# microsoft/ORBIT-Dataset

Hardware: AMD Instinct MI355X
Metric: query frames/sec per task (224×224, 5-way ProtoNet) + frame accuracy vs ref (higher is better)
Workload: dtype f32

## Files before the change

### orbit-dataset_amd/csrc/mbconv_rows.hip

```cpp
#include "bf3.h"
#include "common.h"

namespace orbit {

using f32x16 = __attribute__((ext_vector_type(16))) float;
using v4f = __attribute__((ext_vector_type(4))) float;

using v2f = __attribute__((ext_vector_type(2))) float;

__device__ __forceinline__ v2f silu2(v2f x) {
    const v2f t = x * (v2f){-1.44269502f, -1.44269502f};
    const v2f e = {__builtin_amdgcn_exp2f(t.x), __builtin_amdgcn_exp2f(t.y)};
    const v2f d = e + (v2f){1.0f, 1.0f};
    const v2f r = {__builtin_amdgcn_rcpf(d.x), __builtin_amdgcn_rcpf(d.y)};
    return x * r;
}
__device__ __forceinline__ v2f fma2(v2f a, v2f b, v2f c) { return __builtin_elementwise_fma(a, b, c); }

struct MbRowsParams {
    const float* x;
    const float* w1;
    const float* sc1;
    const float* sh1;
    const float* wdw;
    const float* sc2;
    const float* sh2;
    float* y;
    float* pool;
    int H, W, Cin, mid, pad_t, pad_l, Ho, Wo;
    int SWo, SWi, strips, band_rows, bands, nchunk, total;
};

constexpr int ROWS_ES = 36;

template <int K, int S, int TO, int NOUT, int NG, int SPR, bool EXACT, bool BF3, bool RAW = false>
__global__ __launch_bounds__(256, K == 3 ? 3 : 2) void mbconv_rows3_kernel(const MbRowsParams p) {
    constexpr int NEW = TO * S;
    constexpr int NCOL = (NOUT - 1) * S + K;
    constexpr int ES = ROWS_ES;
    static_assert((TO - 1) * S + K <= 2 * NEW, "an output step reads two windows");
    static_assert(NEW <= 4, "row-in-window index is packed in 2 bits");

    extern __shared__ __attribute__((aligned(16))) float smem[];
    const int n_new = NEW * p.SWi;
    float* ring = smem;

    const int per = gridDim.x >> 3;
    const int v = (blockIdx.x & 7) * per + (blockIdx.x >> 3);
    if (v >= p.total) return;
    const int chunk = v % p.nchunk;
    const int t = v / p.nchunk;
    const int tiles = p.strips * p.bands;
    const int tile = t % tiles, b = t / tiles;
    const int strip = tile % p.strips, band = tile / p.strips;

    const int tid = threadIdx.x, lane = tid & 63;
    const int wave = __builtin_amdgcn_readfirstlane(tid >> 6);
    const int l31 = lane & 31, lh = lane >> 5;
    const int c0 = chunk * 32;
    const int x0 = strip * p.SWo, y0 = band * p.band_rows;
    const int y1 = y0 + p.band_rows < p.Ho ? y0 + p.band_rows : p.Ho;
    const int wi0 = x0 * S - p.pad_l;
    const int r_first = y0 * S - p.pad_t;
    const int NI = (y1 - y0 + TO - 1) / TO;

    const int tstart = wave * 32 < n_new - 32 ? wave * 32 : n_new - 32;
    int a_off, a_rl;
    bool a_colok;
    {
        const int f = tstart + l31;
        a_rl = f / p.SWi;
        const int col = f - a_rl * p.SWi, wi = wi0 + col;
        a_colok = (unsigned)wi < (unsigned)p.W;
        a_off = (a_rl * p.W + wi) * p.Cin + 4 * lh;
    }
    unsigned rowsel[NEW];
#pragma unroll
    for (int r = 0; r < NEW; ++r) rowsel[r] = 0;
#pragma unroll
    for (int e = 0; e < 16; ++e) {
        const int f = tstart + 8 * (e >> 2) + 4 * lh + (e & 3);
        const int rl = f / p.SWi, col = f - rl * p.SWi;
        const bool cok = (unsigned)(wi0 + col) < (unsigned)p.W;
#pragma unroll
        for (int r = 0; r < NEW; ++r)
            if (cok && rl == r) rowsel[r] |= 1u << e;
    }
    v4f wb[NG];
    float s1 = 0.f, h1 = 0.f;
    {
        const int ch = c0 + l31;
#pragma unroll
        for (int g = 0; g < NG; ++g) {
            wb[g] = (v4f){0.f, 0.f, 0.f, 0.f};
            if (ch < p.mid) wb[g] = *reinterpret_cast<const v4f*>(p.w1 + (size_t)ch * p.Cin + 8 * g + 4 * lh);
        }
        if (ch < p.mid) s1 = p.sc1[ch], h1 = p.sh1[ch];
    }
    uint2 wq[BF3 ? 3 : 1][BF3 ? NG : 1];
    if constexpr (BF3) {
#pragma unroll
        for (int g = 0; g < NG; ++g) split3(wb[g], wq[0][g], wq[1][g], wq[2][g]);
    }
    const float* xb = p.x + (size_t)b * p.H * p.W * p.Cin;
    v4f xa[NG];
    auto load_x = [&](int w) {
        const int hi0 = r_first + w * NEW;
        const bool ok = a_colok && (unsigned)(hi0 + a_rl) < (unsigned)p.H;
        const float* src = ok ? xb + (ptrdiff_t)hi0 * p.W * p.Cin + a_off : xb + 4 * lh;
#pragma unroll
        for (int g = 0; g < NG; ++g) xa[g] = *reinterpret_cast<const v4f*>(src + 8 * g);
    };
    float* const Ew0 = ring + tstart * ES + l31;
    auto expand = [&](int w, int slot3) {
        float* Ew = Ew0 + slot3 * n_new * ES;
        const int hi0 = r_first + w * NEW;
        unsigned rowmask = 0;
#pragma unroll
        for (int r = 0; r < NEW; ++r) rowmask |= ((unsigned)(hi0 + r) < (unsigned)p.H ? 1u : 0u) << r;
        f32x16 acc;
#pragma unroll
        for (int r = 0; r < 16; ++r) acc[r] = 0.f;
        if (rowmask != 0) {
            if constexpr (BF3) {
                const uint2 z2 = {0u, 0u};
#pragma unroll
                for (int g = 0; g < NG; g += 2) {
                    uint2 xq[3][2];
                    split3(xa[g], xq[0][0], xq[1][0], xq[2][0]);
                    if (g + 1 < NG) split3(xa[g + 1], xq[0][1], xq[1][1], xq[2][1]);
                    else xq[0][1] = xq[1][1] = xq[2][1] = z2;
                    bf16x8 af[3], bf[3];
#pragma unroll
                    for (int q = 0; q < 3; ++q) {
                        af[q] = bf3_frag(xq[q][0], xq[q][1]);
                        bf[q] = bf3_frag(wq[q][g], g + 1 < NG ? wq[q][g + 1] : z2);
                    }
                    acc = __builtin_amdgcn_mfma_f32_32x32x16_bf16(af[2], bf[0], acc, 0, 0, 0);
                    acc = __builtin_amdgcn_mfma_f32_32x32x16_bf16(af[0], bf[2], acc, 0, 0, 0);
                    acc = __builtin_amdgcn_mfma_f32_32x32x16_bf16(af[1], bf[1], acc, 0, 0, 0);
                    acc = __builtin_amdgcn_mfma_f32_32x32x16_bf16(af[1], bf[0], acc, 0, 0, 0);
                    acc = __builtin_amdgcn_mfma_f32_32x32x16_bf16(af[0], bf[1], acc, 0, 0, 0);
                    acc = __builtin_amdgcn_mfma_f32_32x32x16_bf16(af[0], bf[0], acc, 0, 0, 0);
                }
            } else {
#pragma unroll
                for (int g = 0; g < NG; ++g)
#pragma unroll
                    for (int kk = 0; kk < 4; ++kk) acc = __builtin_amdgcn_mfma_f32_32x32x2f32(xa[g][kk], wb[g][kk], acc, 0, 0, 0);
            }
        }
        load_x(w + 1 <= NI ? w + 1 : NI);
        unsigned okbits = 0;
#pragma unroll
        for (int r = 0; r < NEW; ++r) okbits |= ((rowmask >> r) & 1u) ? rowsel[r] : 0u;
        const v2f s1v = {s1, s1}, h1v = {h1, h1};
        if (__all(okbits == 0xffffu)) {
#pragma unroll
            for (int e = 0; e < 16; e += 2) {
                const v2f val = silu2(fma2((v2f){acc[e], acc[e + 1]}, s1v, h1v));
                Ew[(8 * (e >> 2) + 4 * lh + (e & 3)) * ES] = val.x;
                Ew[(8 * (e >> 2) + 4 * lh + (e & 3) + 1) * ES] = val.y;
            }
        } else {
#pragma unroll
            for (int e = 0; e < 16; e += 2) {
                const v2f val = silu2(fma2((v2f){acc[e], acc[e + 1]}, s1v, h1v));
                const int m0 = __builtin_amdgcn_sbfe((int)okbits, e, 1), m1 = __builtin_amdgcn_sbfe((int)okbits, e + 1, 1);
                const float vx = val.x, vy = val.y;
                Ew[(8 * (e >> 2) + 4 * lh + (e & 3)) * ES] = __int_as_float(__float_as_int(vx) & m0);
                Ew[(8 * (e >> 2) + 4 * lh + (e & 3) + 1) * ES] = __int_as_float(__float_as_int(vy) & m1);
            }
        }
    };

    static_assert(NOUT * S == 2 || NOUT * S == 4, "lane map is built for a 2- or 4-pixel item pitch");
    const unsigned long long CHUNK_MAP = NOUT * S == 2 ? 0xFDCE5764B98A1320ull : 0xFDCE9BA875461320ull;
    const int ck = (int)((CHUNK_MAP >> (4 * (lane >> 2))) & 15u);
    const int lc = ((ck & 1) << 2) | (lane & 3);
    const int u = wave * 8 + (ck >> 1);
    const bool q_real = c0 + lc * 4 < p.mid;
    const int lce = EXACT && !q_real ? lc - 4 : lc;
    const int cq = c0 + lce * 4;
    const bool q_ok = EXACT || q_real;
    static_assert(TO % (32 / SPR) == 0, "a pass covers whole rows of the step");
    v4f s2 = {0.f, 0.f, 0.f, 0.f}, h2 = {0.f, 0.f, 0.f, 0.f};
    if (!RAW && q_ok) s2 = *reinterpret_cast<const v4f*>(p.sc2 + cq), h2 = *reinterpret_cast<const v4f*>(p.sh2 + cq);
    v4f* Ds = reinterpret_cast<v4f*>(ring + 3 * n_new * ES);
    v4f tapr[K == 3 ? K * K : 1];
    if constexpr (K == 3) {
#pragma unroll
        for (int tap = 0; tap < K * K; ++tap)
            tapr[tap] = q_ok ? *reinterpret_cast<const v4f*>(p.wdw + (size_t)tap * p.mid + cq) : (v4f){0.f, 0.f, 0.f, 0.f};
    } else if (tid < K * K * 8) {
        const int tq = c0 + (tid & 7) * 4;
        Ds[tid] = tq < p.mid ? *reinterpret_cast<const v4f*>(p.wdw + (size_t)(tid >> 3) * p.mid + tq) : (v4f){0.f, 0.f, 0.f, 0.f};
    }
    constexpr int RPP = 32 / SPR;
    constexpr int NPASS = (TO + RPP - 1) / RPP;
    const int G = p.SWo / NOUT;
    const int jl = u / SPR, g = u % SPR;
    const int gc = g < G ? g : G - 1;
    const int rowfl = p.SWi * ES;
    const int colpart = gc * (NOUT * S * ES) + lce * 4;
    const int o_col = (x0 + gc * NOUT) * p.mid + cq;
    unsigned okn = 0;
#pragma unroll
    for (int n = 0; n < NOUT; ++n)
        if (g < G && q_ok && x0 + g * NOUT + n < p.Wo) okn |= 1u << n;
    const bool own = g < G && q_real;
    float* ystep = p.y + ((size_t)b * p.Ho + y0) * p.Wo * p.mid;
    const int ystride = TO * p.Wo * p.mid;
    const int orow = p.Wo * p.mid;
    const int band_len = y1 - y0;
    const int winfl = n_new * ES;
    v4f psum = {0.f, 0.f, 0.f, 0.f}, psq = {0.f, 0.f, 0.f, 0.f};

    auto depthwise = [&](int i, int slotA) {
        const int baseA = slotA * winfl;
        const int baseB = slotA == 2 ? 0 : baseA + winfl;
        v2f alo[NOUT], ahi[NOUT];
        v4f cA[NCOL], cB[NCOL];
        auto fetch = [&](v4f* c, int pass, int kh) {
            const float* erow;
            if constexpr (RPP == 1) {
                const int rr = pass * S + kh;
                erow = ring + ((rr >= NEW ? baseB + (rr - NEW) * rowfl : baseA + rr * rowfl) + colpart);
            } else {
                const int rr = (pass * RPP + jl) * S + kh;
                erow = ring + ((rr >= NEW ? baseB - NEW * rowfl : baseA) + __mul24(rr, rowfl) + colpart);
            }
#pragma unroll
            for (int q = 0; q < NCOL; ++q) c[q] = *reinterpret_cast<const v4f*>(erow + q * ES);
        };
        auto mac = [&](const v4f* c, const v4f* t) {
#pragma unroll
            for (int kw = 0; kw < K; ++kw) {
                const v2f flo = {t[kw][0], t[kw][1]}, fhi = {t[kw][2], t[kw][3]};
#pragma unroll
                for (int n = 0; n < NOUT; ++n) {
                    const v4f cv = c[n * S + kw];
                    alo[n] = fma2((v2f){cv[0], cv[1]}, flo, alo[n]);
                    ahi[n] = fma2((v2f){cv[2], cv[3]}, fhi, ahi[n]);
                }
            }
        };
        fetch(cA, 0, 0);
#pragma unroll
        for (int pass = 0; pass < NPASS; ++pass) {
#pragma unroll
            for (int n = 0; n < NOUT; ++n) alo[n] = (v2f){0.f, 0.f}, ahi[n] = (v2f){0.f, 0.f};
            if constexpr (K == 3) {
#pragma unroll
                for (int kh = 0; kh < K; ++kh) {
                    const int f = pass * K + kh;
                    v4f* cur = (f & 1) ? cB : cA;
                    v4f* nxt = (f & 1) ? cA : cB;
                    if (kh + 1 < K) fetch(nxt, pass, kh + 1);
                    else if (pass + 1 < NPASS) fetch(nxt, pass + 1, 0);
                    mac(cur, tapr + kh * K);
                }
            } else {
                static_assert(K == 3 || NPASS == 1, "the 5x5 row loop assumes one pass");
                v4f tA[K], tB[K];
                auto taps = [&](v4f* t, int kh) {
#pragma unroll
                    for (int kw = 0; kw < K; ++kw) t[kw] = Ds[(kh * K + kw) * 8 + lce];
                };
                taps(tA, 0);
#pragma unroll 1
                for (int kh = 0; kh + 1 < K; kh += 2) {
                    fetch(cB, pass, kh + 1), taps(tB, kh + 1);
                    mac(cA, tA);
                    if (kh + 2 < K) fetch(cA, pass, kh + 2), taps(tA, kh + 2);
                    mac(cB, tB);
                }
                if (K & 1) mac(cA, tA);
            }
            const int j = pass * RPP + jl;
            const bool rowok = j < TO && i * TO + j < band_len;
            float* yrow = ystep + j * orow;
#pragma unroll
            for (int n = 0; n < NOUT; ++n) {
                if constexpr (RAW) {
                    const v4f o = {alo[n].x, alo[n].y, ahi[n].x, ahi[n].y};
                    const bool mine = EXACT ? own : (rowok && ((okn >> n) & 1u));
                    if (EXACT || mine) *reinterpret_cast<v4f*>(yrow + (o_col + n * p.mid)) = o;
                    {
#pragma clang fp contract(off)
                        const v4f z = {0.f, 0.f, 0.f, 0.f};
                        psum = psum + (mine ? o : z);
                        psq = psq + (mine ? o * o : z);
                    }
                } else if constexpr (EXACT) {
                    const v2f olo = silu2(fma2(alo[n], (v2f){s2[0], s2[1]}, (v2f){h2[0], h2[1]}));
                    const v2f ohi = silu2(fma2(ahi[n], (v2f){s2[2], s2[3]}, (v2f){h2[2], h2[3]}));
                    const v4f o = {olo.x, olo.y, ohi.x, ohi.y};
                    *reinterpret_cast<v4f*>(yrow + (o_col + n * p.mid)) = o;
                    psum += own ? o : (v4f){0.f, 0.f, 0.f, 0.f};
                } else if (rowok && ((okn >> n) & 1u)) {
                    const v2f olo = silu2(fma2(alo[n], (v2f){s2[0], s2[1]}, (v2f){h2[0], h2[1]}));
                    const v2f ohi = silu2(fma2(ahi[n], (v2f){s2[2], s2[3]}, (v2f){h2[2], h2[3]}));
                    const v4f o = {olo.x, olo.y, ohi.x, ohi.y};
                    *reinterpret_cast<v4f*>(yrow + (o_col + n * p.mid)) = o;
                    {
#pragma clang fp contract(off)
                        psum = psum + o;
                    }
                }
            }
        }
        ystep += ystride;
    };

    load_x(0);
    expand(0, 0);
    expand(1, 1);
    __syncthreads();
    __builtin_amdgcn_s_waitcnt(0x0F70);
    int sa = 0;
    for (int i = 0; i < NI; ++i) {
        if (i + 2 <= NI) expand(i + 2, sa == 0 ? 2 : sa - 1);
        depthwise(i, sa);
        sa = sa == 2 ? 0 : sa + 1;
        __syncthreads();
    }
    if (p.pool) {
        v4f* red = reinterpret_cast<v4f*>(ring);
        red[u * 8 + lc] = psum;
        if constexpr (RAW) red[256 + u * 8 + lc] = psq;
        __syncthreads();
        if (tid < 8 && c0 + tid * 4 < p.mid) {
            v4f t4 = red[tid];
            for (int sl = 1; sl < 32; ++sl) t4 += red[sl * 8 + tid];
            if constexpr (RAW) {
                v4f q4 = red[256 + tid];
                for (int sl = 1; sl < 32; ++sl) q4 += red[256 + sl * 8 + tid];
                float* row = p.pool + ((size_t)b * tiles + tile) * 2 * p.mid + c0 + tid * 4;
                *reinterpret_cast<v4f*>(row) = t4;
                *reinterpret_cast<v4f*>(row + p.mid) = q4;
            } else {
                *reinterpret_cast<v4f*>(p.pool + ((size_t)b * tiles + tile) * p.mid + c0 + tid * 4) = t4;
            }
        }
    }
}

struct RowsGeom {
    int SWo, SWi, strips, band_rows, bands, TO, NOUT;
};
static bool rows_geom(int H, int W, int Cin, int mid, int K, int stride, int Ho, int Wo, RowsGeom& g) {
    if (Cin % 8 != 0 || mid % 4 != 0 || H < 1 || W < 1) return false;
    const int ng = Cin / 8;
    int swo_max = 0;
    if (K == 3 && stride == 2 && ng == 2) g.TO = 1, g.NOUT = 1, swo_max = 28;
    else if (K == 3 && stride == 1 && ng == 3) g.TO = 2, g.NOUT = 2, swo_max = 56;
    else if (K == 5 && stride == 2 && ng == 3) g.TO = 2, g.NOUT = 1, swo_max = 14;
    else if (K == 5 && stride == 1 && ng == 5) g.TO = 4, g.NOUT = 4, swo_max = 28;
    else if (K == 3 && stride == 2 && ng == 5) g.TO = 2, g.NOUT = 1, swo_max = 14;
    else return false;
    g.strips = cdiv(Wo, swo_max);
    g.SWo = cdiv(cdiv(Wo, g.strips), g.NOUT) * g.NOUT;
    g.SWi = (g.SWo - 1) * stride + K;
    const int n_new = g.TO * stride * g.SWi;
    if (n_new <= 32 || n_new > 128) return false;
    g.band_rows = 28;
    g.band_rows = cdiv(g.band_rows, g.TO) * g.TO;
    g.bands = cdiv(Ho, g.band_rows);
    return true;
}

bool mbconv_rows_supported(int H, int W, int Cin, int mid, int K, int stride) {
    RowsGeom g;
    const int Ho = cdiv(H, stride), Wo = cdiv(W, stride);
    return rows_geom(H, W, Cin, mid, K, stride, Ho, Wo, g);
}

int mbconv_rows_tiles(int H, int W, int Cin, int mid, int K, int stride) {
    RowsGeom g;
    const int Ho = cdiv(H, stride), Wo = cdiv(W, stride);
    if (!rows_geom(H, W, Cin, mid, K, stride, Ho, Wo, g)) return 0;
    return g.strips * g.bands;
}

int launch_mbconv_rows(const float* x, const float* w1, const float* sc1, const float* sh1, const float* wdw,
                       const float* sc2, const float* sh2, float* y, float* pool, int B, int H, int W, int Cin, int mid,
                       int K, int stride, int pad_t, int pad_l, int Ho, int Wo, hipStream_t s, int plan_tiles, bool raw_stats) {
    ORBIT_REQUIRE(x && w1 && sc1 && sh1 && wdw && y && (raw_stats ? pool != nullptr : (sc2 && sh2)), "mbconv_rows: null pointer");
    RowsGeom g;
    ORBIT_REQUIRE(Ho == cdiv(H, stride) && Wo == cdiv(W, stride) && rows_geom(H, W, Cin, mid, K, stride, Ho, Wo, g),
                  "mbconv_rows: unsupported shape (H=%d W=%d Cin=%d mid=%d K=%d s=%d)", H, W, Cin, mid, K, stride);
    ORBIT_REQUIRE(plan_tiles <= 0 || plan_tiles == g.strips * g.bands,
                  "mbconv_rows: the plan was built for %d pooling tiles per frame, this launch writes %d", plan_tiles, g.strips * g.bands);
    MbRowsParams p;
    p.x = x, p.w1 = w1, p.sc1 = sc1, p.sh1 = sh1, p.wdw = wdw, p.sc2 = sc2, p.sh2 = sh2, p.y = y, p.pool = pool;
    p.H = H, p.W = W, p.Cin = Cin, p.mid = mid, p.pad_t = pad_t, p.pad_l = pad_l, p.Ho = Ho, p.Wo = Wo;
    p.SWo = g.SWo, p.SWi = g.SWi, p.strips = g.strips, p.band_rows = g.band_rows, p.bands = g.bands;
    p.nchunk = cdiv(mid, 32);
    p.total = p.nchunk * g.strips * g.bands * B;
    const int grid = cdiv(p.total, 8) * 8;
    const int n_new = g.TO * stride * g.SWi;
    const size_t lds = (size_t)3 * n_new * ROWS_ES * sizeof(float) + (K == 3 ? 0 : (size_t)K * K * 8 * 16);
    const double pix = (double)B * H * W;
    const int rec = prof_start(raw_stats ? "mbconv_rows,raw" : "mbconv_rows", 2.0 * pix * Cin * mid + 2.0 * B * Ho * Wo * mid * K * K,
                               4.0 * (pix * Cin + (double)B * Ho * Wo * mid), s, pix * mid + (raw_stats ? 0.0 : (double)B * Ho * Wo * mid));
#define ORBIT_MBR3(KK, SS, TO_, NOUT_, NG_, SPR_, EX_, BF_)                                                       \
    do {                                                                                                \
        if (raw_stats) {                                                                                \
            if constexpr (!BF_) {                                                                       \
                auto kern = mbconv_rows3_kernel<KK, SS, TO_, NOUT_, NG_, SPR_, EX_, false, true>;           \
                static bool attr_set = false;                                                           \
                if (!attr_set) {                                                                        \
                    ORBIT_HIP_CHECK(hipFuncSetAttribute(reinterpret_cast<const void*>(kern),            \
                                                        hipFuncAttributeMaxDynamicSharedMemorySize, 64 * 1024)); \
                    attr_set = true;                                                                    \
                }                                                                                       \
                kern<<<grid, 256, lds, s>>>(p);                                                         \
            }                                                                                           \
            break;                                                                                      \
        }                                                                                               \
        auto kern = mbconv_rows3_kernel<KK, SS, TO_, NOUT_, NG_, SPR_, EX_, BF_>;                                \
        static bool attr_set = false;                                                                   \
        if (!attr_set) {                                                                                \
            ORBIT_HIP_CHECK(hipFuncSetAttribute(reinterpret_cast<const void*>(kern),                    \
                                                hipFuncAttributeMaxDynamicSharedMemorySize, 64 * 1024)); \
            attr_set = true;                                                                            \
        }                                                                                               \
        kern<<<grid, 256, lds, s>>>(p);                                                                 \
    } while (0)
    const int ng = Cin / 8;
    const bool exact = g.strips * g.SWo == Wo && Ho % g.TO == 0 && g.band_rows % g.TO == 0 && (mid % 32 == 0 || mid % 32 == 16) &&
                       g.SWo % g.NOUT == 0;
    const bool bf3 = !raw_stats && (get_option("conv_bf3") & 2) != 0;
#define ORBIT_MBR3X(KK, SS, TO_, NOUT_, NG_, SPR_)                    \
    do {                                                              \
        if (exact && bf3) ORBIT_MBR3(KK, SS, TO_, NOUT_, NG_, SPR_, true, true);   \
        else if (exact) ORBIT_MBR3(KK, SS, TO_, NOUT_, NG_, SPR_, true, false);    \
        else ORBIT_MBR3(KK, SS, TO_, NOUT_, NG_, SPR_, false, false);              \
    } while (0)
    if (K == 3 && stride == 2 && ng == 2) ORBIT_MBR3X(3, 2, 1, 1, 2, 32);
    else if (K == 3 && stride == 1 && ng == 3) ORBIT_MBR3X(3, 1, 2, 2, 3, 32);
    else if (K == 5 && stride == 2 && ng == 3) ORBIT_MBR3X(5, 2, 2, 1, 3, 16);
    else if (K == 5 && stride == 1 && ng == 5) ORBIT_MBR3X(5, 1, 4, 4, 5, 8);
    else if (exact) ORBIT_MBR3(3, 2, 2, 1, 5, 16, true, false);
    else ORBIT_MBR3(3, 2, 2, 1, 5, 16, false, false);
#undef ORBIT_MBR3X
#undef ORBIT_MBR3
    prof_stop(rec, s);
    ORBIT_LAUNCH_CHECK();
    return ORBIT_OK;
}


struct StemRowsParams {
    const float* frames;
    const float* w1;
    const float* sc1;
    const float* sh1;
    const float* wdw;
    const float* sc2;
    const float* sh2;
    float* y;
    float* pool;
    int FH, FW, spad_t, spad_l, H, W;
    int SWo, SWi, strips, band_rows, bands, total;
};

constexpr int STEM_PW = 64;

template <bool EXACT>
__global__ __launch_bounds__(256, 3) void stem_rows_kernel(const StemRowsParams p, const float* __restrict__ w1g,
                                                           const float* __restrict__ sc1g, const float* __restrict__ sh1g) {
    constexpr int K = 3, TO = 2, NEW = 2, NOUT = 2, NCOL = 4, ES = ROWS_ES;
    extern __shared__ __attribute__((aligned(16))) float smem[];
    const int n_new = NEW * p.SWi;
    float* ring = smem;
    float* patch = ring + 3 * n_new * ES;
    constexpr int PATCH = 3 * 5 * STEM_PW;

    const int per = gridDim.x >> 3;
    const int v = (blockIdx.x & 7) * per + (blockIdx.x >> 3);
    if (v >= p.total) return;
    const int tiles = p.strips * p.bands;
    const int tile = v % tiles, b = v / tiles;
    const int strip = tile % p.strips, band = tile / p.strips;
    const int tid = threadIdx.x, lane = tid & 63;
    const int wave = __builtin_amdgcn_readfirstlane(tid >> 6);
    const int x0 = strip * p.SWo, y0 = band * p.band_rows;
    const int y1 = y0 + p.band_rows < p.H ? y0 + p.band_rows : p.H;
    const int c_first = x0 - 1, r_first = y0 - 1;
    const int NI = (y1 - y0 + TO - 1) / TO;
    const float* fb = p.frames + (size_t)b * 3 * p.FH * p.FW;

    const int fcol0 = 2 * c_first - p.spad_l;
    const int pcols = 2 * p.SWi + 1;
    constexpr int NPL = (PATCH + 255) / 256;
    float preg[NPL];
    unsigned pmask = 0;
    int poff[NPL];
    unsigned pcolok = 0, prows = 0;
#pragma unroll
    for (int u = 0; u < NPL; ++u) {
        const int i = tid + u * 256;
        const int c = i & (STEM_PW - 1), pr = i >> 6;
        const int plane = pr / 5, row = pr - plane * 5;
        const int fc = fcol0 + c;
        const bool cok = i < PATCH && c < pcols && (unsigned)fc < (unsigned)p.FW;
        poff[u] = cok ? (plane * p.FH + row) * p.FW + fc : 0;
        pcolok |= (cok ? 1u : 0u) << u;
        prows |= (unsigned)row << (3 * u);
    }
    auto patch_load = [&](int w) {
        const int frow0 = 2 * (r_first + NEW * w) - p.spad_t;
        unsigned rmask = 0;
#pragma unroll
        for (int r = 0; r < 5; ++r) rmask |= ((unsigned)(frow0 + r) < (unsigned)p.FH ? 1u : 0u) << r;
        const int rowbase = frow0 * p.FW;
        pmask = 0;
#pragma unroll
        for (int u = 0; u < NPL; ++u) {
            const bool ok = ((pcolok >> u) & 1u) && ((rmask >> ((prows >> (3 * u)) & 7u)) & 1u);
            pmask |= (ok ? 1u : 0u) << u;
            preg[u] = fb[ok ? poff[u] + rowbase : 0];
        }
    };
    auto patch_store = [&](int w) {
        float* dst = patch + (w & 1) * PATCH;
#pragma unroll
        for (int u = 0; u < NPL; ++u) {
            const int i = tid + u * 256;
            if (i < PATCH) dst[i] = ((pmask >> u) & 1u) ? preg[u] : 0.f;
        }
    };

    using f32x4 = __attribute__((ext_vector_type(4))) float;
    const int l15 = lane & 15, lq = lane >> 4;
    float* Wl = patch + 2 * PATCH;
    for (int i = tid; i < 14 * 64; i += 256) {
        const int ln = i & 63, hs = i >> 6, h = hs / 7, st = hs - h * 7;
        const int k = 4 * st + (ln >> 4);
        Wl[i] = k < 27 ? w1g[(16 * h + (ln & 15)) * 32 + k] : 0.f;
    }
    int a_base;
    {
        const int fa = wave * 16 + l15 < n_new ? wave * 16 + l15 : n_new - 1;
        const int rl = fa / p.SWi, col = fa - rl * p.SWi;
        a_base = (2 * rl) * STEM_PW + 2 * col;
    }
    float s1c[2], h1c[2];
#pragma unroll
    for (int h = 0; h < 2; ++h) s1c[h] = sc1g[16 * h + l15], h1c[h] = sh1g[16 * h + l15];
    unsigned o_inwin = 0, sel0 = 0, sel1 = 0;
#pragma unroll
    for (int r = 0; r < 4; ++r) {
        const int fo = wave * 16 + 4 * lq + r;
        const int rl = fo / p.SWi, col = fo - rl * p.SWi;
        if (fo < n_new) o_inwin |= 1u << r;
        if (fo < n_new && (unsigned)(c_first + col) < (unsigned)p.W) (rl ? sel1 : sel0) |= 1u << r;
    }
    auto stem = [&](int w) {
        const float* P = patch + (w & 1) * PATCH + a_base;
        f32x4 acc0 = {0.f, 0.f, 0.f, 0.f}, acc1 = {0.f, 0.f, 0.f, 0.f};
#pragma unroll
        for (int st = 0; st < 7; ++st) {
            const int k = 4 * st + lq < 27 ? 4 * st + lq : 0;
            const int ci = k / 9, kh = (k - ci * 9) / 3, kw = k - ci * 9 - kh * 3;
            const float av = P[(ci * 5 + kh) * STEM_PW + kw];
            acc0 = __builtin_amdgcn_mfma_f32_16x16x4f32(av, Wl[st * 64 + lane], acc0, 0, 0, 0);
            acc1 = __builtin_amdgcn_mfma_f32_16x16x4f32(av, Wl[(7 + st) * 64 + lane], acc1, 0, 0, 0);
        }
        const int hi0 = r_first + NEW * w;
        const unsigned okbits = ((unsigned)hi0 < (unsigned)p.H ? sel0 : 0u) | ((unsigned)(hi0 + 1) < (unsigned)p.H ? sel1 : 0u);
        float* E = ring + ((w % 3) * n_new + wave * 16 + 4 * lq) * ES + l15;
#pragma unroll
        for (int r = 0; r < 4; r += 2) {
            const v2f v0 = silu2(fma2((v2f){acc0[r], acc0[r + 1]}, (v2f){s1c[0], s1c[0]}, (v2f){h1c[0], h1c[0]}));
            const v2f v1 = silu2(fma2((v2f){acc1[r], acc1[r + 1]}, (v2f){s1c[1], s1c[1]}, (v2f){h1c[1], h1c[1]}));
            const float a0 = v0.x, a1 = v0.y, b0 = v1.x, b1 = v1.y;
            const int m0 = __builtin_amdgcn_sbfe((int)okbits, r, 1), m1 = __builtin_amdgcn_sbfe((int)okbits, r + 1, 1);
            if ((o_inwin >> r) & 1u) {
                E[r * ES] = __int_as_float(__float_as_int(a0) & m0);
                E[r * ES + 16] = __int_as_float(__float_as_int(b0) & m0);
            }
            if ((o_inwin >> (r + 1)) & 1u) {
                E[(r + 1) * ES] = __int_as_float(__float_as_int(a1) & m1);
                E[(r + 1) * ES + 16] = __int_as_float(__float_as_int(b1) & m1);
            }
        }
    };

    const unsigned long long CHUNK_MAP = 0xFDCE5764B98A1320ull;
    const int ck = (int)((CHUNK_MAP >> (4 * (lane >> 2))) & 15u);
    const int lc = ((ck & 1) << 2) | (lane & 3);
    const int u = wave * 8 + (ck >> 1);
    const int cq = lc * 4;
    const v4f s2 = *reinterpret_cast<const v4f*>(p.sc2 + cq), h2 = *reinterpret_cast<const v4f*>(p.sh2 + cq);
    v4f tapr[K * K];
#pragma unroll
    for (int tap = 0; tap < K * K; ++tap) tapr[tap] = *reinterpret_cast<const v4f*>(p.wdw + tap * 32 + cq);
    const int G = p.SWo / NOUT;
    const int jl = u >> 4, g = u & 15;
    const int gc = g < G ? g : G - 1;
    const int rowfl = p.SWi * ES, winfl = n_new * ES;
    const int colpart = gc * (NOUT * ES) + lc * 4;
    const int o_col = (jl * p.W + x0 + gc * NOUT) * 32 + cq;
    const bool own = g < G;
    unsigned okn = 0;
#pragma unroll
    for (int n = 0; n < NOUT; ++n)
        if (g < G && x0 + g * NOUT + n < p.W) okn |= 1u << n;
    float* ystep = p.y + ((size_t)b * p.H + y0) * p.W * 32;
    const int band_len = y1 - y0;
    v4f psum = {0.f, 0.f, 0.f, 0.f};
    auto depthwise = [&](int i, int slotA) {
        const int baseA = slotA * winfl;
        const int baseB = slotA == 2 ? 0 : baseA + winfl;
        v2f alo[NOUT], ahi[NOUT];
#pragma unroll
        for (int n = 0; n < NOUT; ++n) alo[n] = (v2f){0.f, 0.f}, ahi[n] = (v2f){0.f, 0.f};
        v4f cA[NCOL], cB[NCOL];
        auto fetch = [&](v4f* c, int kh) {
            const int rr = jl + kh;
            const float* erow = ring + ((rr >= NEW ? baseB - NEW * rowfl : baseA) + __mul24(rr, rowfl) + colpart);
#pragma unroll
            for (int q = 0; q < NCOL; ++q) c[q] = *reinterpret_cast<const v4f*>(erow + q * ES);
        };
        fetch(cA, 0);
#pragma unroll
        for (int kh = 0; kh < K; ++kh) {
            v4f* cur = (kh & 1) ? cB : cA;
            v4f* nxt = (kh & 1) ? cA : cB;
            if (kh + 1 < K) fetch(nxt, kh + 1);
#pragma unroll
            for (int kw = 0; kw < K; ++kw) {
                const v4f t = tapr[kh * K + kw];
                const v2f flo = {t[0], t[1]}, fhi = {t[2], t[3]};
#pragma unroll
                for (int n = 0; n < NOUT; ++n) {
                    const v4f cv = cur[n + kw];
                    alo[n] = fma2((v2f){cv[0], cv[1]}, flo, alo[n]);
                    ahi[n] = fma2((v2f){cv[2], cv[3]}, fhi, ahi[n]);
                }
            }
        }
        const bool rowok = i * TO + jl < band_len;
#pragma unroll
        for (int n = 0; n < NOUT; ++n) {
            if constexpr (EXACT) {
                const v2f olo = silu2(fma2(alo[n], (v2f){s2[0], s2[1]}, (v2f){h2[0], h2[1]}));
                const v2f ohi = silu2(fma2(ahi[n], (v2f){s2[2], s2[3]}, (v2f){h2[2], h2[3]}));
                const v4f o = {olo.x, olo.y, ohi.x, ohi.y};
                *reinterpret_cast<v4f*>(ystep + (o_col + n * 32)) = o;
                psum += own ? o : (v4f){0.f, 0.f, 0.f, 0.f};
            } else if (rowok && ((okn >> n) & 1u)) {
                const v2f olo = silu2(fma2(alo[n], (v2f){s2[0], s2[1]}, (v2f){h2[0], h2[1]}));
                const v2f ohi = silu2(fma2(ahi[n], (v2f){s2[2], s2[3]}, (v2f){h2[2], h2[3]}));
                const v4f o = {olo.x, olo.y, ohi.x, ohi.y};
                *reinterpret_cast<v4f*>(ystep + (o_col + n * 32)) = o;
                {
#pragma clang fp contract(off)
                    psum = psum + o;
                }
            }
        }
        ystep += TO * p.W * 32;
    };

    patch_load(0);
    patch_store(0);
    __syncthreads();
    __builtin_amdgcn_s_waitcnt(0x0F70);
    int sa = 0;
    for (int w = 0; w <= NI + 1; ++w) {
        patch_load(w + 1 <= NI ? w + 1 : NI);
        if (w <= NI) stem(w);
        if (w >= 2) {
            depthwise(w - 2, sa);
            sa = sa == 2 ? 0 : sa + 1;
        }
        if (w + 1 <= NI) patch_store(w + 1);
        __syncthreads();
    }
    if (p.pool) {
        v4f* red = reinterpret_cast<v4f*>(ring);
        red[u * 8 + lc] = psum;
        __syncthreads();
        if (tid < 8) {
            v4f t4 = red[tid];
            for (int sl = 1; sl < 32; ++sl) t4 += red[sl * 8 + tid];
            *reinterpret_cast<v4f*>(p.pool + ((size_t)b * tiles + tile) * 32 + tid * 4) = t4;
        }
    }
}

struct StemRowsGeom {
    int SWo, SWi, strips, band_rows, bands;
};
static bool stem_rows_geom(int H, int W, int mid, int K, int stride, StemRowsGeom& g) {
    if (mid != 32 || K != 3 || stride != 1 || H < 1 || W < 1) return false;
    g.strips = cdiv(W, 28);
    g.SWo = cdiv(cdiv(W, g.strips), 2) * 2;
    g.SWi = g.SWo + 2;
    if (2 * g.SWi > 64) return false;
    g.band_rows = 28;
    g.band_rows = cdiv(g.band_rows, 2) * 2;
    g.bands = cdiv(H, g.band_rows);
    return true;
}
bool stem_rows_supported(int H, int W, int mid, int K, int stride) {
    StemRowsGeom g;
    return stem_rows_geom(H, W, mid, K, stride, g);
}
int stem_rows_tiles(int H, int W) {
    StemRowsGeom g;
    return stem_rows_geom(H, W, 32, 3, 1, g) ? g.strips * g.bands : 0;
}

int launch_stem_rows(const float* frames, const float* w1_packed, const float* sc1, const float* sh1, const float* wdw,
                     const float* sc2, const float* sh2, float* y, float* pool, int B, int FH, int FW, int spad_t,
                     int spad_l, int H, int W, hipStream_t s, int plan_tiles) {
    ORBIT_REQUIRE(frames && w1_packed && sc1 && sh1 && wdw && sc2 && sh2 && y, "stem_rows: null pointer");
    StemRowsGeom g;
    ORBIT_REQUIRE(stem_rows_geom(H, W, 32, 3, 1, g), "stem_rows: unsupported shape (H=%d W=%d)", H, W);
    ORBIT_REQUIRE(plan_tiles <= 0 || plan_tiles == g.strips * g.bands,
                  "stem_rows: the plan was built for %d pooling tiles per frame, this launch writes %d", plan_tiles, g.strips * g.bands);
    StemRowsParams p;
    p.frames = frames, p.w1 = w1_packed, p.sc1 = sc1, p.sh1 = sh1, p.wdw = wdw, p.sc2 = sc2, p.sh2 = sh2, p.y = y, p.pool = pool;
    p.FH = FH, p.FW = FW, p.spad_t = spad_t, p.spad_l = spad_l, p.H = H, p.W = W;
    p.SWo = g.SWo, p.SWi = g.SWi, p.strips = g.strips, p.band_rows = g.band_rows, p.bands = g.bands;
    p.total = g.strips * g.bands * B;
    const int grid = cdiv(p.total, 8) * 8;
    const size_t lds = ((size_t)3 * 2 * g.SWi * ROWS_ES + 2 * 3 * 5 * STEM_PW + 14 * 64) * sizeof(float);
    const double pix = (double)B * H * W;
    const int rec = prof_start("stem_rows", 2.0 * pix * 32 * 27 + 2.0 * pix * 32 * 9,
                               4.0 * ((double)B * 3 * FH * FW + pix * 32), s, 2.0 * pix * 32);
    if (g.strips * g.SWo == W && H % 2 == 0 && g.band_rows % 2 == 0) stem_rows_kernel<true><<<grid, 256, lds, s>>>(p, w1_packed, sc1, sh1);
    else stem_rows_kernel<false><<<grid, 256, lds, s>>>(p, w1_packed, sc1, sh1);
    prof_stop(rec, s);
    ORBIT_LAUNCH_CHECK();
    return ORBIT_OK;
}

__global__ __launch_bounds__(256) void stem_pack_kernel(const float* __restrict__ w, float* __restrict__ wp, int mid) {
    for (int i = blockIdx.x * 256 + threadIdx.x; i < mid * 32; i += gridDim.x * 256) {
        const int r = i >> 5, k = i & 31;
        wp[i] = k < 27 ? w[r * 27 + k] : 0.f;
    }
}
int stem_pack_weights(const float* w_oihw, float* w_packed, int mid, hipStream_t s) {
    stem_pack_kernel<<<cdiv(mid * 32, 256), 256, 0, s>>>(w_oihw, w_packed, mid);
    ORBIT_LAUNCH_CHECK();
    return ORBIT_OK;
}

}

using namespace orbit;

extern "C" int orbit_op_stem_dw_front_partials(int H, int W, int mid) {
    return stem_rows_supported(H, W, mid, 3, 1) ? stem_rows_tiles(H, W) : 0;
}

extern "C" int orbit_op_stem_dw_front(const float* frames, const float* w_stem, const float* scale1, const float* shift1,
                                      const float* wdw, const float* scale2, const float* shift2, float* y,
                                      float* pool_partial, int B, int FH, int FW, int spad_top, int spad_left, int H, int W,
                                      int mid, int pad_top, int pad_left, int Ho, int Wo, orbit_stream_t stream) {
    ORBIT_REQUIRE(frames && w_stem && wdw && y, "op_stem_dw_front: null pointer");
    ORBIT_REQUIRE(stem_rows_supported(H, W, mid, 3, 1) && pad_top == 1 && pad_left == 1 && Ho == H && Wo == W,
                  "op_stem_dw_front: unsupported shape (H=%d W=%d mid=%d)", H, W, mid);
    hipStream_t s = (hipStream_t)stream;
    float* wp = nullptr;
    ORBIT_HIP_CHECK(hipMallocAsync(reinterpret_cast<void**>(&wp), (size_t)mid * (32 + 9) * sizeof(float), s));
    int rc = stem_pack_weights(w_stem, wp, mid, s);
    if (rc == ORBIT_OK) rc = dwconv_pack_weights(wdw, wp + (size_t)mid * 32, mid, 3, s);
    if (rc == ORBIT_OK)
        rc = launch_stem_rows(frames, wp, scale1, shift1, wp + (size_t)mid * 32, scale2, shift2, y, pool_partial, B, FH, FW,
                              spad_top, spad_left, H, W, s);
    (void)hipFreeAsync(wp, s);
    return rc;
}

extern "C" int orbit_op_mbconv_front_partials(int H, int W, int Cin, int mid, int K, int stride) {
    return mbconv_rows_supported(H, W, Cin, mid, K, stride) ? mbconv_rows_tiles(H, W, Cin, mid, K, stride) : 0;
}

extern "C" int orbit_op_mbconv_front(const float* x, const float* w1, const float* scale1, const float* shift1,
                                     const float* wdw, const float* scale2, const float* shift2, float* y,
                                     float* pool_partial, int B, int H, int W, int Cin, int mid, int K, int stride,
                                     int pad_top, int pad_left, int Ho, int Wo, orbit_stream_t stream) {
    ORBIT_REQUIRE(x && w1 && wdw && y, "op_mbconv_front: null pointer");
    ORBIT_REQUIRE(mbconv_rows_supported(H, W, Cin, mid, K, stride),
                  "op_mbconv_front: unsupported shape (H=%d W=%d Cin=%d mid=%d K=%d s=%d)", H, W, Cin, mid, K, stride);
    hipStream_t s = (hipStream_t)stream;
    float* wp = nullptr;
    ORBIT_HIP_CHECK(hipMallocAsync(reinterpret_cast<void**>(&wp), (size_t)mid * K * K * sizeof(float), s));
    int rc = dwconv_pack_weights(wdw, wp, mid, K, s);
    if (rc == ORBIT_OK)
        rc = launch_mbconv_rows(x, w1, scale1, shift1, wp, scale2, shift2, y, pool_partial, B, H, W, Cin, mid, K, stride,
                                pad_top, pad_left, Ho, Wo, s);
    (void)hipFreeAsync(wp, s);
    return rc;
}
```

Baseline: 37720.

## Vectorize stem patch loads and keep stem weights in registers

Adds a VEC variant of the stem kernel. It loads each input patch row as aligned float4 segments, shifting the patch origin to a 4-element boundary, instead of issuing several scalar loads per thread. Stem weights are now held in per-lane registers rather than staged through LDS, which removes the LDS weight buffer and its fill loop. The per-step patch offsets are precomputed, and all A operands are loaded before the MFMA chain. The trade is higher register use under launch_bounds(256,3), and the aligned path only runs when FW is a multiple of 4 and the frame pointer is 16-byte aligned.

New measurement: 37790 (median of 6 runs). About the same (+0.2%).

```diff
diff --git a/orbit-dataset_amd/csrc/mbconv_rows.hip b/orbit-dataset_amd/csrc/mbconv_rows.hip
--- a/orbit-dataset_amd/csrc/mbconv_rows.hip
+++ b/orbit-dataset_amd/csrc/mbconv_rows.hip
@@ -468,7 +468,7 @@
 
 constexpr int STEM_PW = 64;
 
-template <bool EXACT>
+template <bool EXACT, bool VEC>
 __global__ __launch_bounds__(256, 3) void stem_rows_kernel(const StemRowsParams p, const float* __restrict__ w1g,
                                                            const float* __restrict__ sc1g, const float* __restrict__ sh1g) {
     constexpr int K = 3, TO = 2, NEW = 2, NOUT = 2, NCOL = 4, ES = ROWS_ES;
@@ -494,24 +494,42 @@
 
     const int fcol0 = 2 * c_first - p.spad_l;
     const int pcols = 2 * p.SWi + 1;
-    constexpr int NPL = (PATCH + 255) / 256;
+    const int shift = VEC ? (fcol0 & 3) : 0;
+    constexpr int NPL = VEC ? 1 : (PATCH + 255) / 256;
     float preg[NPL];
+    v4f pvec = {0.f, 0.f, 0.f, 0.f};
     unsigned pmask = 0;
     int poff[NPL];
     unsigned pcolok = 0, prows = 0;
-#pragma unroll
-    for (int u = 0; u < NPL; ++u) {
-        const int i = tid + u * 256;
-        const int c = i & (STEM_PW - 1), pr = i >> 6;
+    if constexpr (VEC) {
+        const int seg = tid & 15, pr = tid >> 4;
         const int plane = pr / 5, row = pr - plane * 5;
-        const int fc = fcol0 + c;
-        const bool cok = i < PATCH && c < pcols && (unsigned)fc < (unsigned)p.FW;
-        poff[u] = cok ? (plane * p.FH + row) * p.FW + fc : 0;
-        pcolok |= (cok ? 1u : 0u) << u;
-        prows |= (unsigned)row << (3 * u);
+        const int fc = fcol0 - shift + 4 * seg;
+        const bool cok = pr < 15 && (unsigned)fc < (unsigned)p.FW;
+        poff[0] = cok ? (plane * p.FH + row) * p.FW + fc : 0;
+        pcolok = cok ? 1u : 0u;
+        prows = (unsigned)row;
+    } else {
+#pragma unroll
+        for (int u = 0; u < NPL; ++u) {
+            const int i = tid + u * 256;
+            const int c = i & (STEM_PW - 1), pr = i >> 6;
+            const int plane = pr / 5, row = pr - plane * 5;
+            const int fc = fcol0 + c;
+            const bool cok = i < PATCH && c < pcols && (unsigned)fc < (unsigned)p.FW;
+            poff[u] = cok ? (plane * p.FH + row) * p.FW + fc : 0;
+            pcolok |= (cok ? 1u : 0u) << u;
+            prows |= (unsigned)row << (3 * u);
+        }
     }
     auto patch_load = [&](int w) {
         const int frow0 = 2 * (r_first + NEW * w) - p.spad_t;
+        if constexpr (VEC) {
+            const bool ok = pcolok && (unsigned)(frow0 + (int)prows) < (unsigned)p.FH;
+            pmask = ok ? 1u : 0u;
+            pvec = *reinterpret_cast<const v4f*>(fb + (ok ? poff[0] + frow0 * p.FW : 0));
+            return;
+        }
         unsigned rmask = 0;
 #pragma unroll
         for (int r = 0; r < 5; ++r) rmask |= ((unsigned)(frow0 + r) < (unsigned)p.FH ? 1u : 0u) << r;
@@ -526,6 +544,10 @@
     };
     auto patch_store = [&](int w) {
         float* dst = patch + (w & 1) * PATCH;
+        if constexpr (VEC) {
+            if (tid < PATCH / 4) *reinterpret_cast<v4f*>(dst + 4 * tid) = pmask ? pvec : (v4f){0.f, 0.f, 0.f, 0.f};
+            return;
+        }
 #pragma unroll
         for (int u = 0; u < NPL; ++u) {
             const int i = tid + u * 256;
@@ -535,17 +557,24 @@
 
     using f32x4 = __attribute__((ext_vector_type(4))) float;
     const int l15 = lane & 15, lq = lane >> 4;
-    float* Wl = patch + 2 * PATCH;
-    for (int i = tid; i < 14 * 64; i += 256) {
-        const int ln = i & 63, hs = i >> 6, h = hs / 7, st = hs - h * 7;
-        const int k = 4 * st + (ln >> 4);
-        Wl[i] = k < 27 ? w1g[(16 * h + (ln & 15)) * 32 + k] : 0.f;
+    float wr0[7], wr1[7];
+#pragma unroll
+    for (int st = 0; st < 7; ++st) {
+        wr0[st] = w1g[l15 * 32 + 4 * st + lq];
+        wr1[st] = w1g[(16 + l15) * 32 + 4 * st + lq];
     }
     int a_base;
     {
         const int fa = wave * 16 + l15 < n_new ? wave * 16 + l15 : n_new - 1;
         const int rl = fa / p.SWi, col = fa - rl * p.SWi;
-        a_base = (2 * rl) * STEM_PW + 2 * col;
+        a_base = (2 * rl) * STEM_PW + 2 * col + shift;
+    }
+    int a_off[7];
+#pragma unroll
+    for (int st = 0; st < 7; ++st) {
+        const int k = 4 * st + lq < 27 ? 4 * st + lq : 0;
+        const int ci = k / 9, kh = (k - ci * 9) / 3, kw = k - ci * 9 - kh * 3;
+        a_off[st] = a_base + (ci * 5 + kh) * STEM_PW + kw;
     }
     float s1c[2], h1c[2];
 #pragma unroll
@@ -559,15 +588,15 @@
         if (fo < n_new && (unsigned)(c_first + col) < (unsigned)p.W) (rl ? sel1 : sel0) |= 1u << r;
     }
     auto stem = [&](int w) {
-        const float* P = patch + (w & 1) * PATCH + a_base;
+        const float* P = patch + (w & 1) * PATCH;
         f32x4 acc0 = {0.f, 0.f, 0.f, 0.f}, acc1 = {0.f, 0.f, 0.f, 0.f};
+        float av[7];
+#pragma unroll
+        for (int st = 0; st < 7; ++st) av[st] = P[a_off[st]];
 #pragma unroll
         for (int st = 0; st < 7; ++st) {
-            const int k = 4 * st + lq < 27 ? 4 * st + lq : 0;
-            const int ci = k / 9, kh = (k - ci * 9) / 3, kw = k - ci * 9 - kh * 3;
-            const float av = P[(ci * 5 + kh) * STEM_PW + kw];
-            acc0 = __builtin_amdgcn_mfma_f32_16x16x4f32(av, Wl[st * 64 + lane], acc0, 0, 0, 0);
-            acc1 = __builtin_amdgcn_mfma_f32_16x16x4f32(av, Wl[(7 + st) * 64 + lane], acc1, 0, 0, 0);
+            acc0 = __builtin_amdgcn_mfma_f32_16x16x4f32(av[st], wr0[st], acc0, 0, 0, 0);
+            acc1 = __builtin_amdgcn_mfma_f32_16x16x4f32(av[st], wr1[st], acc1, 0, 0, 0);
         }
         const int hi0 = r_first + NEW * w;
         const unsigned okbits = ((unsigned)hi0 < (unsigned)p.H ? sel0 : 0u) | ((unsigned)(hi0 + 1) < (unsigned)p.H ? sel1 : 0u);
@@ -730,12 +759,17 @@
     p.SWo = g.SWo, p.SWi = g.SWi, p.strips = g.strips, p.band_rows = g.band_rows, p.bands = g.bands;
     p.total = g.strips * g.bands * B;
     const int grid = cdiv(p.total, 8) * 8;
-    const size_t lds = ((size_t)3 * 2 * g.SWi * ROWS_ES + 2 * 3 * 5 * STEM_PW + 14 * 64) * sizeof(float);
+    const size_t lds = ((size_t)3 * 2 * g.SWi * ROWS_ES + 2 * 3 * 5 * STEM_PW) * sizeof(float);
     const double pix = (double)B * H * W;
     const int rec = prof_start("stem_rows", 2.0 * pix * 32 * 27 + 2.0 * pix * 32 * 9,
-                               4.0 * ((double)B * 3 * FH * FW + pix * 32), s, 2.0 * pix * 32);
-    if (g.strips * g.SWo == W && H % 2 == 0 && g.band_rows % 2 == 0) stem_rows_kernel<true><<<grid, 256, lds, s>>>(p, w1_packed, sc1, sh1);
-    else stem_rows_kernel<false><<<grid, 256, lds, s>>>(p, w1_packed, sc1, sh1);
+                               4.0 * ((double)B * 3 * FH * FW + pix * 32 + (pool ? (double)B * g.strips * g.bands * 32 : 0.0)), s,
+                               2.0 * pix * 32);
+    const bool exact = g.strips * g.SWo == W && H % 2 == 0 && g.band_rows % 2 == 0;
+    const bool vec = FW % 4 == 0 && reinterpret_cast<uintptr_t>(frames) % 16 == 0;
+    if (exact && vec) stem_rows_kernel<true, true><<<grid, 256, lds, s>>>(p, w1_packed, sc1, sh1);
+    else if (exact) stem_rows_kernel<true, false><<<grid, 256, lds, s>>>(p, w1_packed, sc1, sh1);
+    else if (vec) stem_rows_kernel<false, true><<<grid, 256, lds, s>>>(p, w1_packed, sc1, sh1);
+    else stem_rows_kernel<false, false><<<grid, 256, lds, s>>>(p, w1_packed, sc1, sh1);
     prof_stop(rec, s);
     ORBIT_LAUNCH_CHECK();
     return ORBIT_OK;
```
